# Liozou/CrystalEnergyGrids.jl

Measured on AMD Instinct MI355X. Metric: grid-points/sec, higher is better.
Workload: dtype f64; 1 GPU; CHA_1.4_3b4eeb96 tiled 2x2x3 (11664 atoms) x 256^3 grid, Ar probe LJ + real-space Ewald; grid_points=16777216, framework_atoms=11664, lattice_images=37460, mode=fused, algo=culled, parallelism=x-slab sharding over 1 GPU(s)

## Files before the change

### crystalenergygrids.jl_amd/csrc/ceg_kernels.hip

```cpp
#include <type_traits>

#include "ceg_internal.h"
#include "ceg_math.h"
#include "ceg_minimage.h"

namespace ceg {

struct Accum {
    double v, d1x, d1y, d1z, d2xy, d2xz, d2yz, d3;
};

__device__ __forceinline__ void accum_zero(Accum& a)
{
    a.v = a.d1x = a.d1y = a.d1z = a.d2xy = a.d2xz = a.d2yz = a.d3 = 0.0;
}

__device__ __forceinline__ void accum_add(Accum& a, double v, double p1, double p2, double p3,
                                          double dx, double dy, double dz)
{
    a.v += v;
    a.d1x += p1 * dx;
    a.d1y += p1 * dy;
    a.d1z += p1 * dz;
    const double d13 = dx * dz;
    a.d2xy += p2 * (dx * dy);
    a.d2xz += p2 * d13;
    a.d2yz += p2 * (dy * dz);
    a.d3 += p3 * d13 * dy;
}

__device__ __forceinline__ double grid_coord(int i, double size, int dims, double shift)
{
#pragma clang fp contract(off)
    return __dadd_rn(__ddiv_rn(__dmul_rn((double)i, size), (double)dims), shift);
}

__device__ __attribute__((noinline)) double exp_out_of_line(double x) { return exp(x); }

template <bool LJONLY = false, bool COLD = false>
__device__ __forceinline__ void vdw_terms(const DevRule* __restrict__ rules, int rb, int re, double r2,
                                          double& v_out, double& p1_out, double& p2_out, double& p3_out)
{
    double v = 0.0, p1 = 0.0, p2 = 0.0, p3 = 0.0;
    for (int t = rb; t < re; ++t) {
        const int kind = rules[t].kind;
        const double q0 = rules[t].p0, q1 = rules[t].p1, q2 = rules[t].p2, sh = rules[t].shift;
        double tv, t1 = 0.0, t2 = 0.0, t3 = 0.0;
        if (LJONLY || kind == CEG_LENNARDJONES) {
            const double inv = 1.0 / r2;
            const double s = q1 * inv;
            const double x6 = s * s * s;
            const double inv2 = inv * inv;
            tv = 4.0 * q0 * x6 * (x6 - 1.0);
            t1 = 24.0 * q0 * (x6 * (1.0 - 2.0 * x6)) * inv;
            t2 = 96.0 * q0 * (x6 * (7.0 * x6 - 2.0)) * inv2;
            t3 = 384.0 * q0 * (x6 * (5.0 - 28.0 * x6)) * (inv2 * inv2);
        } else if (kind == CEG_BUCKINGHAM) {
            const double A = q0, B = q1, C = q2;
            const double r4 = r2 * r2;
            const double r = sqrt(r2);
            const double r6 = r4 * r2;
            const double x6 = C / r6;
            const double xe = A * (COLD ? exp_out_of_line(-B * r) : exp(-B * r));
            tv = xe - x6;
            t1 = -B * xe / r + 6.0 * x6 / r2;
            t2 = -48.0 * x6 / r4 + B * xe * (1.0 + B * r) / (r2 * r);
            t3 = -(3.0 * B * r + B * B * r2 + 3.0) * B * xe * r / r6 + 480.0 * C / (r6 * r6);
        } else {
            tv = (r2 < q0) ? __builtin_huge_val() : 0.0;
        }
        v += tv - sh;
        p1 += t1;
        p2 += t2;
        p3 += t3;
    }
    v_out = v; p1_out = p1; p2_out = p2; p3_out = p3;
}

__device__ __forceinline__ void ewald_terms(double alpha, double charge, double r2,
                                            double& v, double& p1, double& p2, double& p3)
{
    const double inv_sqrtpi = 0.56418958354775628695;
    const double r = sqrt(r2);
    const double r3 = r2 * r;
    const double r5 = r3 * r2;
    const double r2a2 = r2 * (alpha * alpha);
    const double er2a2 = 2.0 * alpha * r * exp(-r2a2) * inv_sqrtpi;
    const double erfar = erfc(alpha * r);
    v = charge * erfar / r;
    p1 = -charge * (er2a2 + erfar) / r3;
    p2 = charge * (er2a2 * (3.0 + 2.0 * r2a2) + 3.0 * erfar) / r5;
    p3 = charge * (-er2a2 * (15.0 + 10.0 * r2a2 + 4.0 * (r2a2 * r2a2)) - 15.0 * erfar) / (r5 * r2);
}

__device__ __forceinline__ void ewald_terms_poly(double alpha, double charge, double r2,
                                                 double& v, double& p1, double& p2, double& p3)
{
    const double inv_sqrtpi = 0.56418958354775628695;
    const double r = sqrt(r2);
    const double r3 = r2 * r;
    const double r5 = r3 * r2;
    const double r2a2 = r2 * (alpha * alpha);
    const double E = fast_exp_neg(-r2a2);
    const double er2a2 = 2.0 * alpha * r * E * inv_sqrtpi;
    const double erfar = E * erfcx_poly(alpha * r);
    v = charge * erfar / r;
    p1 = -charge * (er2a2 + erfar) / r3;
    p2 = charge * (er2a2 * (3.0 + 2.0 * r2a2) + 3.0 * erfar) / r5;
    p3 = charge * (-er2a2 * (15.0 + 10.0 * r2a2 + 4.0 * (r2a2 * r2a2)) - 15.0 * erfar) / (r5 * r2);
}

__device__ __attribute__((noinline)) double4 ewald_terms_poly_call(double alpha, double charge, double r2)
{
    double v, p1, p2, p3;
    ewald_terms_poly(alpha, charge, r2, v, p1, p2, p3);
    return make_double4(v, p1, p2, p3);
}
__device__ __attribute__((noinline)) double4 lj_terms_call(const DevRule* __restrict__ rules, int rb, int re, double r2)
{
    double v, p1, p2, p3;
    vdw_terms<true, true>(rules, rb, re, r2, v, p1, p2, p3);
    return make_double4(v, p1, p2, p3);
}

__device__ __forceinline__ double clamp_julia(double x, double lo, double hi)
{
    return (x > hi) ? hi : ((x < lo) ? lo : x);
}

__device__ __forceinline__ void store_gridpoint(float* __restrict__ out, int64_t idx, int64_t cs,
                                                const double* delta, double lambda, double thr, Accum a)
{
#pragma clang fp contract(off)
    if (a.v > thr) {
        a.v = 2.0 * thr;
        a.d1x = clamp_julia(a.d1x, -thr, thr);
        a.d1y = clamp_julia(a.d1y, -thr, thr);
        a.d1z = clamp_julia(a.d1z, -thr, thr);
        a.d2xy = a.d2xz = a.d2yz = 0.0;
        a.d3 = 0.0;
    }
    const double D1 = delta[0], D2 = delta[1], D3 = delta[2];
    out[idx] = (float)__dmul_rn(a.v, lambda);
    out[idx + cs] = (float)__dmul_rn(__dmul_rn(a.d1x, D1), lambda);
    out[idx + 2 * cs] = (float)__dmul_rn(__dmul_rn(a.d1y, D2), lambda);
    out[idx + 3 * cs] = (float)__dmul_rn(__dmul_rn(a.d1z, D3), lambda);
    out[idx + 4 * cs] = (float)__dmul_rn(__dmul_rn(a.d2xy, __dmul_rn(D1, D2)), lambda);
    out[idx + 5 * cs] = (float)__dmul_rn(__dmul_rn(a.d2xz, __dmul_rn(D1, D3)), lambda);
    out[idx + 6 * cs] = (float)__dmul_rn(__dmul_rn(a.d2yz, __dmul_rn(D2, D3)), lambda);
    out[idx + 7 * cs] = (float)__dmul_rn(__dmul_rn(a.d3, __dmul_rn(__dmul_rn(D1, D2), D3)), lambda);
}

__device__ __forceinline__ void gridpoint8(float r[8], const double* delta, double lambda, double thr, Accum a)
{
#pragma clang fp contract(off)
    if (a.v > thr) {
        a.v = 2.0 * thr;
        a.d1x = clamp_julia(a.d1x, -thr, thr);
        a.d1y = clamp_julia(a.d1y, -thr, thr);
        a.d1z = clamp_julia(a.d1z, -thr, thr);
        a.d2xy = a.d2xz = a.d2yz = 0.0;
        a.d3 = 0.0;
    }
    const double D1 = delta[0], D2 = delta[1], D3 = delta[2];
    r[0] = (float)__dmul_rn(a.v, lambda);
    r[1] = (float)__dmul_rn(__dmul_rn(a.d1x, D1), lambda);
    r[2] = (float)__dmul_rn(__dmul_rn(a.d1y, D2), lambda);
    r[3] = (float)__dmul_rn(__dmul_rn(a.d1z, D3), lambda);
    r[4] = (float)__dmul_rn(__dmul_rn(a.d2xy, __dmul_rn(D1, D2)), lambda);
    r[5] = (float)__dmul_rn(__dmul_rn(a.d2xz, __dmul_rn(D1, D3)), lambda);
    r[6] = (float)__dmul_rn(__dmul_rn(a.d2yz, __dmul_rn(D2, D3)), lambda);
    r[7] = (float)__dmul_rn(__dmul_rn(a.d3, __dmul_rn(__dmul_rn(D1, D2), D3)), lambda);
}

typedef float ceg_v4f __attribute__((ext_vector_type(4)));
__device__ __forceinline__ void store_float4_unaligned(float* dst, float4 v)
{
    const ceg_v4f u = {v.x, v.y, v.z, v.w};
    asm volatile("global_store_dwordx4 %0, %1, off" : : "v"(dst), "v"(u) : "memory");
}

__device__ __forceinline__ void store_raw(double* __restrict__ out, int64_t p, const Accum& a)
{
    double* o = out + 8 * p;
    o[0] = a.v;  o[1] = a.d1x;  o[2] = a.d1y;  o[3] = a.d1z;
    o[4] = a.d2xy;  o[5] = a.d2xz;  o[6] = a.d2yz;  o[7] = a.d3;
}

// ... 128 lines not shown
           : (mode == 2 && vdwk >= 2 && ewk) ? CEG_WAVES_FUSED_BUCK
           : (mode == 2 && vdwk == 1 && ewk) ? CEG_WAVES_FUSED_LJ
           : (mode == 0 && vdwk == 1)      ? CEG_WAVES_VDW_LJ
           : (mode == 0 && vdwk >= 2)      ? CEG_WAVES_VDW_BUCK
           : (mode == 1 && ewk)            ? CEG_WAVES_COULOMB
                                           : CEG_WAVES;
}
#ifndef CEG_NW_EW2
#define CEG_NW_EW2 8
#endif
constexpr int culled_nw(int mode, int vdwk, int ewk, int np = 1)
{
    return np > 1 ? (mode == 2 ? CEG_NW_MULTI_FUSED : CEG_WG / 64)
                  : ((mode != 0 && ewk == 2) || (mode != 1 && vdwk == 3)) ? CEG_NW_EW2 : CEG_WG / 64;
}
[[maybe_unused]] constexpr double R_EXACT2 = CEG_R_EXACT2;
static_assert(ERFCX_TAB_N == CEG_ERFCX_TAB_N, "table size mismatch");
constexpr int META_SIMPLE = 1 << 24;
constexpr int META_HASVDW = 1 << 25;
constexpr int META_BUCK = 1 << 26;
constexpr int META_KINDMASK = (1 << 24) - 1;

struct __attribute__((aligned(16))) Quad { double x, y, z, w; };
struct __attribute__((aligned(16))) CandRec {
    Quad xyzq;
    Quad lj;
    int32_t meta;
    int32_t atom;
    int32_t _pad[2];
};

template <int MODE, bool FASTEW, bool LJSLOW, bool EWSCALED, bool BKSCALED, int NP, int UNI = 0, bool DOV = true, bool DOC = true, typename Rec>
__device__ __forceinline__ void slow_pairs(const PlanConst* __restrict__ pc, unsigned long long cands, int lane,
                                           double px, double py, double pz,
                                           const Rec* s_rec,
                                           const unsigned long long* s_odd,
                                           Accum* avm, const int32_t* probe_idx, Accum& ac, double& smallest_d2)
{
    Accum& av = avm[0];
    const Geom& g = pc->g;
    while (cands != 0ull) {
        const int q = __builtin_ctzll(cands);
        cands &= cands - 1ull;
        const unsigned long long lanes = s_odd[q];
        if (!((lanes >> lane) & 1ull)) continue;
        const int mt = s_rec[q].meta;
        const double4 O = pc->ib.atoms[s_rec[q].atom];
        double dx = px - O.x, dy = py - O.y, dz = pz - O.z;
        const double r2 = periodic_distance2_literal(g, dx, dy, dz);
        if (r2 >= g.cutoff2) continue;
        if constexpr (NP > 1) {
            if (DOV && (mt & META_HASVDW)) {
                const int kd = mt & META_KINDMASK;
#pragma unroll
                for (int p = 0; p < NP; ++p) {
                    const RuleTable& rtp = pc->rtm[probe_idx[p]];
                    const int rb = rtp.offset[kd], re = rtp.offset[kd + 1];
                    if (re == rb) continue;
                    const double4 T = lj_terms_call(rtp.rules, rb, re, r2);
                    accum_add(avm[p], T.x, T.y * (-1.0 / 6.0), T.z * (1.0 / 48.0), T.w * (-1.0 / 480.0), dx, dy, dz);
                }
            }
        } else if (MODE != MODE_COULOMB && (mt & META_HASVDW)) {
            const int kd = mt & META_KINDMASK;
            double v, p1, p2, p3;
            vdw_terms<LJSLOW, true>(pc->rt.rules, pc->rt.offset[kd], pc->rt.offset[kd + 1], r2, v, p1, p2, p3);
            if (UNI) {
                v *= pc->uni_sv; p1 *= pc->uni_s1; p2 *= pc->uni_s2; p3 *= pc->uni_s3;
            } else if (LJSLOW) {
                p1 *= -1.0 / 6.0; p2 *= 1.0 / 48.0; p3 *= -1.0 / 480.0;
            }
            if (BKSCALED) {
                v *= pc->bk_invC; p1 *= pc->bk_s1; p2 *= pc->bk_s2; p3 *= pc->bk_s3;
            }
            accum_add(av, v, p1, p2, p3, dx, dy, dz);
        }
        if (MODE != MODE_VDW && DOC) {
            smallest_d2 = fmin(smallest_d2, r2);
            double v, p1, p2, p3;
            if constexpr (NP > 1) {
                const double4 T = ewald_terms_poly_call(g.alpha, O.w, r2);
                v = T.x; p1 = T.y; p2 = T.z; p3 = T.w;
            } else if (FASTEW)
                ewald_terms_poly(g.alpha, O.w, r2, v, p1, p2, p3);
            else
                ewald_terms(g.alpha, O.w, r2, v, p1, p2, p3);
            if (UNI == 2) {
                v *= pc->uni_inv_q; p1 *= pc->uni_inv_q; p2 *= pc->uni_qs2; p3 *= pc->uni_qs3;
            } else if (EWSCALED) {
                p2 *= 1.0 / 3.0; p3 *= 1.0 / 15.0;
            }
            accum_add(ac, v, p1, p2, p3, dx, dy, dz);
        }
    }
}

__device__ __forceinline__ int mad_u24(int a, int b, int c)
{
    int r;
    asm("v_mad_u32_u24 %0, %1, %2, %3" : "=v"(r) : "v"(a), "v"(b), "s"(c));
    return r;
}

__device__ __forceinline__ double uniform(double x)
{
    int lo = __double2loint(x), hi = __double2hiint(x);
    asm("" : "+v"(lo));
    asm("" : "+v"(hi));
    return __hiloint2double(__builtin_amdgcn_readfirstlane(hi), __builtin_amdgcn_readfirstlane(lo));
}

__device__ __forceinline__ double wave_min(double x)
{
#pragma unroll
    for (int o = 32; o > 0; o >>= 1) x = fmin(x, __shfl_xor(x, o));
    return x;
}
__device__ __forceinline__ double wave_max(double x)
{
#pragma unroll
    for (int o = 32; o > 0; o >>= 1) x = fmax(x, __shfl_xor(x, o));
    return x;
}

static_assert(sizeof(CandRec) == 80, "candidate record layout");
struct __attribute__((aligned(16))) CandRecS {
    Quad xyzq;
    int32_t meta;
    int32_t atom;
    int32_t _pad[2];
};
static_assert(sizeof(CandRecS) == 48, "candidate record layout");
template <int NP>
struct __attribute__((aligned(16))) CandRecM {
    Quad xyzq;
    double ljm[3 * NP + (NP & 1)];
    int32_t meta;
    int32_t atom;
    int32_t _pad[2];
};
static_assert(sizeof(CandRecM<2>) == 96 && sizeof(CandRecM<3>) == 128 && sizeof(CandRecM<4>) == 144, "candidate record layout");
template <int NP> __device__ __forceinline__ Quad lj_record(const CandRecM<NP>& r, int p) { return Quad{r.ljm[3 * p], 0.0, r.ljm[3 * p + 1], r.ljm[3 * p + 2]}; }
__device__ __forceinline__ Quad lj_record(const CandRec& r, int) { return r.lj; }
__device__ __forceinline__ Quad lj_record(const CandRecS&, int) { return Quad{0.0, 0.0, 0.0, 0.0}; }
template <int NP> __device__ __forceinline__ void set_lj_record(CandRecM<NP>& r, int p, Quad q) { r.ljm[3 * p] = q.x; r.ljm[3 * p + 1] = q.z; r.ljm[3 * p + 2] = q.w; }
__device__ __forceinline__ void set_lj_record(CandRec& r, int, Quad q) { r.lj = q; }
__device__ __forceinline__ void set_lj_record(CandRecS&, int, Quad) {}

template <int MODE, bool POINTS, int VDWK, int EWK, int NP = 1>
__global__ __launch_bounds__(64 * culled_nw(MODE, VDWK, EWK, NP), culled_waves(MODE, VDWK, EWK, NP)) void k_culled(const PlanConst* __restrict__ pc, Output out, Points pts,
                                                              int tiles_j, int tiles_k, int64_t ntiles)
{
    static_assert(NP >= 1 && NP <= CEG_MAX_PROBES && (NP == 1 || (VDWK == 1 && !POINTS && EWK == 2 && MODE != MODE_COULOMB)), "multi-probe variant");
    constexpr bool MULTI = NP > 1;
    constexpr bool FASTEW = EWK != 0;
    constexpr bool EW2 = EWK == 2 && MODE != MODE_VDW;
    constexpr int WG = 64 * culled_nw(MODE, VDWK, EWK, NP);
    constexpr bool BK2 = VDWK == 3 && MODE != MODE_COULOMB;
    constexpr bool UNI = vdwk_uniform(VDWK) && MODE != MODE_COULOMB;
    constexpr bool UNIQ = VDWK == 5 && MODE == MODE_FUSED && EWK == 2;
    static_assert(!vdwk_uniform(VDWK) || (NP == 1 && MODE != MODE_COULOMB && (VDWK == 4 || UNIQ)), "uniform variants");
    constexpr int NW = WG / 64;
    constexpr bool HAS_LJ = !MULTI && (VDWK == 1 || VDWK == 2) && MODE != MODE_COULOMB;
    using Rec = std::conditional_t<MULTI, CandRecM<NP>, std::conditional_t<HAS_LJ, CandRec, CandRecS>>;
    __shared__ __attribute__((aligned(16))) Rec s_rec_all[NW][64];
    __shared__ int32_t s_rowstart_all[NW][64];
    __shared__ int32_t s_rowprefix_all[NW][66];
    __shared__ unsigned long long s_odd_all[NW][64];
    __shared__ __attribute__((aligned(16))) double s_erfcx[EW2 ? 2 : ERFCX_TAB_N * 6];
    constexpr int EW2_LS = (NP == 1) ? CEG_EW2_LDS_STRIDE : CEG_EW2_STRIDE;
    __shared__ __attribute__((aligned(16))) double s_ew2[EW2 ? CEG_EW2_NI_MAX * EW2_LS : 2];
    __shared__ __attribute__((aligned(16))) double s_bk2[BK2 ? CEG_BK2_NI_MAX * CEG_BK2_STRIDE : 2];
    __shared__ double s_exp2[64];
    __shared__ int32_t s_org[NW][4];

    const int wave = __builtin_amdgcn_readfirstlane(threadIdx.x >> 6);
    Rec* s_rec = s_rec_all[wave];
    int32_t* s_rowstart = s_rowstart_all[wave];
    int32_t* s_rowprefix = s_rowprefix_all[wave];
    unsigned long long* s_odd = s_odd_all[wave];

    constexpr bool FASTVDW = VDWK != 0;
    if (EW2) {
        const int nt = pc->ew2_ni * CEG_EW2_STRIDE;
        for (int t = threadIdx.x; t < nt; t += WG) s_ew2[(t / CEG_EW2_STRIDE) * EW2_LS + t % CEG_EW2_STRIDE] = pc->ew2_tab[t];
    } else if (FASTEW && MODE != MODE_VDW) {
        for (int t = threadIdx.x; t < ERFCX_TAB_N * 6; t += WG) s_erfcx[t] = pc->erfcx_tab[t];
    }
    if (BK2) {
        const int nt = pc->bk2_ni * CEG_BK2_STRIDE;
        for (int t = threadIdx.x; t < nt; t += WG) s_bk2[t] = pc->bk2_tab[t];
    }
    if ((FASTEW && !EW2 && MODE != MODE_VDW) || (VDWK == 2 && MODE != MODE_COULOMB))
        if (threadIdx.x < 64) s_exp2[threadIdx.x] = pc->exp2_tab[threadIdx.x];
    __syncthreads();
    const int64_t tile_raw = (int64_t)blockIdx.x * NW + wave;
    const bool active = tile_raw < ntiles;
    const int64_t tile = active ? tile_raw : ntiles - 1;

    const Geom& g = pc->g;
    const ImageBins& ib = pc->ib;
    const RuleTable& rt = pc->rt;
    const int lane = threadIdx.x & 63;
    const double cutoff2 = g.cutoff2;
    const double r_exact2 = pc->r_exact2;
    const double alpha = g.alpha;
    const int32_t ortho = g.ortho;
    const double safemin2 = g.safemin2;

    int i = 0, j = 0, k = 0;
    int i0 = 0, j0 = 0, k0 = 0;
    int64_t pidx = 0;
    bool valid;
    double px, py, pz;
    if (POINTS) {
        pidx = tile * 64 + lane;
        valid = active && pidx < pts.n;
        const int64_t tt = valid ? pidx : (pts.n - 1);
        px = pts.xyz[3 * tt]; py = pts.xyz[3 * tt + 1]; pz = pts.xyz[3 * tt + 2];
    } else {
        const int tj = (int)((tile / tiles_k) % tiles_j);
        const int ti = (int)(tile / ((int64_t)tiles_k * tiles_j));
        const int nq = (tiles_k + NW - 1) / NW;
        const int tk = (int)((tile % tiles_k + (int64_t)NW * ((ti + (out.i_begin >> 2) + tj) % nq)) % tiles_k);
        i0 = out.i_begin + 4 * ti; j0 = 4 * tj; k0 = 4 * tk;
        if (lane == 0) {
            s_org[wave][0] = active ? i0 : -1;
            s_org[wave][1] = j0;
            s_org[wave][2] = k0;
        }
        i = i0 + (lane >> 4);
        j = j0 + ((lane >> 2) & 3);
        k = k0 + (lane & 3);
        valid = active && (i < out.i_end) && (j <= g.dims[1]) && (k <= g.dims[2]);
        const int ci = i < out.i_end ? i : out.i_end - 1;
        const int cj = j <= g.dims[1] ? j : g.dims[1];
        const int ck = k <= g.dims[2] ? k : g.dims[2];
        px = grid_coord(ci, g.size[0], g.dims[0], g.shift[0]);
        py = grid_coord(cj, g.size[1], g.dims[1], g.shift[1]);
        pz = grid_coord(ck, g.size[2], g.dims[2], g.shift[2]);
    }

    const double blx = uniform(wave_min(px)), bhx = uniform(wave_max(px));
    const double bly = uniform(wave_min(py)), bhy = uniform(wave_max(py));
    const double blz = uniform(wave_min(pz)), bhz = uniform(wave_max(pz));
    const double cx = uniform(0.5 * (blx + bhx)), cy = uniform(0.5 * (bly + bhy)), cz = uniform(0.5 * (blz + bhz));
    const double hx = uniform(0.5 * (bhx - blx)), hy = uniform(0.5 * (bhy - bly)), hz = uniform(0.5 * (bhz - blz));
    const double rc2 = uniform(cutoff2 * (1.0 + 1e-9) + 1e-9);
    const double rc = uniform(sqrt(rc2));

    auto bin_of = [&](double x, int ax) -> int {
        int b = (int)floor((x - ib.lo[ax]) * ib.inv_bin[ax]);
        b = b < 0 ? 0 : b;
        return b >= ib.nb[ax] ? ib.nb[ax] - 1 : b;
    };
    const int bx0 = bin_of(blx - rc, 0), bx1 = bin_of(bhx + rc, 0);
    const int by0 = bin_of(bly - rc, 1), by1 = bin_of(bhy + rc, 1);
    const int nry = by1 - by0 + 1;
    const int nrows = active ? (bx1 - bx0 + 1) * nry : 0;
    const float inv_nry = __int_as_float(__builtin_amdgcn_readfirstlane(__float_as_int(1.0f / (float)nry)));

    Accum avm[NP], ac;
#pragma unroll
    for (int p = 0; p < NP; ++p) accum_zero(avm[p]);
    Accum& av = avm[0];
    accum_zero(ac);
    double smallest_d2 = __builtin_huge_val();
    const double band_cut = 1e-9 * cutoff2;
    const double alpha2 = pc->alpha2;
    const bool stale_possible = !ortho && safemin2 < cutoff2;
    const double cut_hi = uniform(cutoff2 + band_cut);
    const double reg_hi = uniform(stale_possible ? fmin(cutoff2 - band_cut, safemin2 * (1.0 - 1e-9)) : cutoff2 - band_cut);
    const double erf_inv_h = pc->erfcx_inv_h, erf_mx0 = pc->erfcx_mx0_inv_h;
    const int hi_lo = __builtin_amdgcn_readfirstlane(__double2hiint(r_exact2) + (__double2loint(r_exact2) != 0 ? 1 : 0));
    const int hi_top = __builtin_amdgcn_readfirstlane(__double2hiint(reg_hi));
    const unsigned hi_span = hi_top > hi_lo ? (unsigned)(hi_top - hi_lo) : 0u;
    const int hi_cut = __builtin_amdgcn_readfirstlane(__double2hiint(cut_hi));
    const double int_lo = uniform(r_exact2 * (1.0 + 4e-6)), int_hi = uniform(reg_hi * (1.0 - 4e-6));
    const int ew2_off = EW2 ? __builtin_amdgcn_readfirstlane(-pc->ew2_base * (EW2_LS * 8)) : 0;
    int ew2_stride = EW2_LS * 8;
    asm volatile("" : "+v"(ew2_stride));
    const double ew_k3 = pc->ew_k3, ew_k15 = pc->ew_k15;
    const bool all_simple = __builtin_amdgcn_readfirstlane(pc->all_simple) != 0;
    const int bk2_off = BK2 ? __builtin_amdgcn_readfirstlane(-pc->bk2_base * (CEG_BK2_STRIDE * 8)) : 0;
    int bk2_stride = CEG_BK2_STRIDE * 8;
    asm volatile("" : "+v"(bk2_stride));
    const double uni_s6 = UNI ? uniform(pc->uni_s6) : 0.0, uni_k1 = UNI ? uniform(pc->uni_k1) : 0.0;
    const double uni_k2 = UNI ? uniform(pc->uni_k2) : 0.0, uni_k3 = UNI ? uniform(pc->uni_k3) : 0.0;
    const double uni_inv_q = UNIQ ? uniform(pc->uni_inv_q) : 0.0;
    int uni_count = 0;
    int uni_count_all = 0;
    const double bk_B = pc->bk_B, bk_nshift = pc->bk_nshift, bk_c1 = pc->bk_c1, bk_c2 = pc->bk_c2, bk_c3 = pc->bk_c3, bk_c4 = pc->bk_c4;

    for (int rbase = 0; rbase < nrows; rbase += 64) {
        int count = 0, start = 0;
        const int r = rbase + lane;
        if (r < nrows) {
            const int rq = (int)(((float)r + 0.5f) * inv_nry);
            const int bx = bx0 + rq, by = by0 + (r - rq * nry);
            const double colx0 = ib.lo[0] + bx * ib.bin[0], colx1 = colx0 + ib.bin[0];
            const double coly0 = ib.lo[1] + by * ib.bin[1], coly1 = coly0 + ib.bin[1];
            const double gx = fmax(0.0, fmax(blx - colx1, colx0 - bhx));
            const double gy = fmax(0.0, fmax(bly - coly1, coly0 - bhy));
            const double dxy2 = gx * gx + gy * gy;
            if (dxy2 < rc2) {
                const double zr = sqrt(rc2 - dxy2);
                const int bz0 = bin_of(blz - zr, 2), bz1 = bin_of(bhz + zr, 2);
                const int64_t rowbase = ((int64_t)bx * ib.nb[1] + by) * ib.nb[2];
                start = ib.bin_start[rowbase + bz0];
                count = ib.bin_start[rowbase + bz1 + 1] - start;
            }
        }
        int ln = lane;
        asm volatile("" : "+v"(ln));
        int incl = count;
#pragma unroll
        for (int o = 1; o < 64; o <<= 1) {
            const int up = __builtin_amdgcn_ds_bpermute((ln - o) << 2, incl);
            if (ln >= o) incl += up;
        }
        __builtin_amdgcn_wave_barrier();
        s_rowstart[ln] = start;
        s_rowprefix[ln + 1] = incl;
        if (ln == 0) s_rowprefix[0] = 0;
        __builtin_amdgcn_wave_barrier();
        const int total = __builtin_amdgcn_readfirstlane(s_rowprefix[64]);

        for (int cbase = 0; cbase < total; cbase += 64) {
            const int t = cbase + lane;
            bool keep = false, interior = false;
            double4 P = make_double4(0, 0, 0, 0);
            double4 LJ = make_double4(0, 0, 0, 0);
            double4 LJM[NP];
#pragma unroll
            for (int p = 0; p < NP; ++p) LJM[p] = make_double4(0, 0, 0, 0);
            int meta = 0, aidx = 0;
            if (t < total) {
                int lo = 0, hi = 64;
#pragma unroll
                for (int s = 0; s < 6; ++s) {
                    const int mid = (lo + hi) >> 1;
                    if (s_rowprefix[mid] <= t) lo = mid; else hi = mid;
                }
                const int img = s_rowstart[lo] + (t - s_rowprefix[lo]);
                P = ib.xyzq[img];
                aidx = ib.atom[img];
                const int kw = ib.kind ? ib.kind[img] : -1;
                const int kd = kw < 0 ? -1 : (kw & META_KINDMASK);
                const double qx = fmax(0.0, fabs(cx - P.x) - hx);
                const double qy = fmax(0.0, fabs(cy - P.y) - hy);
                const double qz = fmax(0.0, fabs(cz - P.z) - hz);
                const double dmin2 = qx * qx + qy * qy + qz * qz;
                keep = dmin2 < rc2;
                const double fx = fabs(cx - P.x) + hx, fy = fabs(cy - P.y) + hy, fz = fabs(cz - P.z) + hz;
                interior = dmin2 > int_lo && (fx * fx + fy * fy + fz * fz) < int_hi;
                bool hasvdw = false;
                int vclass = 0;
                if (MODE != MODE_COULOMB && kd >= 0) {
                    hasvdw = (kw & META_HASVDW) != 0;
                    if constexpr (MULTI) {
                        if (hasvdw && keep) {
#pragma unroll
                            for (int p = 0; p < NP; ++p) {
                                const FastVdw F = pc->fastm[out.probe_idx[p]][kd];
                                LJM[p] = make_double4(F.p0, F.p1, F.p2, F.shift);
                            }
                        }
                    } else if (FASTVDW && VDWK != 3 && !UNI && hasvdw && keep) {
                        const FastVdw F = pc->fastvdw[kd];
                        LJ = make_double4(F.p0, F.p1, F.p2, F.shift);
                        vclass = F.cls;
                    }
                }
                if (MODE == MODE_VDW) keep = keep && hasvdw;
                bool simple = g.diag != 0 || (!POINTS && all_simple);
                if (!simple && keep) {
                    const double* I = g.invmat;
                    const double ux = cx - P.x, uy = cy - P.y, uz = cz - P.z;
                    const double f0 = I[0] * ux + I[3] * uy + I[6] * uz;
                    const double f1 = I[1] * ux + I[4] * uy + I[7] * uz;
                    const double f2 = I[2] * ux + I[5] * uy + I[8] * uz;
                    const double e0 = fabs(I[0]) * hx + fabs(I[3]) * hy + fabs(I[6]) * hz + 1e-9;
                    const double e1 = fabs(I[1]) * hx + fabs(I[4]) * hy + fabs(I[7]) * hz + 1e-9;
                    const double e2 = fabs(I[2]) * hx + fabs(I[5]) * hy + fabs(I[8]) * hz + 1e-9;
                    simple = (fabs(f0) + e0 < 0.5) && (fabs(f1) + e1 < 0.5) && (fabs(f2) + e2 < 0.5);
                }
                meta = (kd & META_KINDMASK) | (simple ? META_SIMPLE : 0) | (hasvdw ? META_HASVDW : 0) |
                       (vclass == 2 ? META_BUCK : 0);
            }
#ifdef CEG_SKIP_TESTS
            keep = keep && (P.x == 12345.678);
#endif
            const bool simple_c = (meta & META_SIMPLE) != 0;
            const bool withv = MODE != MODE_COULOMB && (meta & META_HASVDW) != 0;
            const bool ks = keep && simple_c;
            const unsigned long long mask_vi = __builtin_amdgcn_ballot_w64(ks && withv && interior);
            const unsigned long long mask_vb = __builtin_amdgcn_ballot_w64(ks && withv && !interior);
            const unsigned long long mask_ni = __builtin_amdgcn_ballot_w64(ks && !withv && interior);
            const unsigned long long mask_nb = __builtin_amdgcn_ballot_w64(ks && !withv && !interior);
            const unsigned long long mask_x = __builtin_amdgcn_ballot_w64(keep && !simple_c);
            const int nvi = __popcll(mask_vi), nv = nvi + __popcll(mask_vb), nni = nv + __popcll(mask_ni), nreg = nni + __popcll(mask_nb),
                      nkeep = nreg + __popcll(mask_x);
            __builtin_amdgcn_wave_barrier();
            if (keep) {
                const unsigned long long mine = !simple_c ? mask_x : (withv ? (interior ? mask_vi : mask_vb) : (interior ? mask_ni : mask_nb));
                const int first = !simple_c ? nreg : (withv ? (interior ? 0 : nvi) : (interior ? nv : nni));
                const int slot = first + __builtin_amdgcn_mbcnt_hi((unsigned)(mine >> 32), __builtin_amdgcn_mbcnt_lo((unsigned)mine, 0));
                s_rec[slot].xyzq = Quad{P.x, P.y, P.z, (UNIQ && !withv) ? mul_sc(P.w, uni_inv_q) : P.w};
                if constexpr (MULTI) {
#pragma unroll
                    for (int p = 0; p < NP; ++p) set_lj_record(s_rec[slot], p, Quad{LJM[p].x, LJM[p].y, LJM[p].z, LJM[p].w});
                } else if constexpr (HAS_LJ) s_rec[slot].lj = Quad{LJ.x, LJ.y, LJ.z, LJ.w};
                s_rec[slot].meta = meta;
                s_rec[slot].atom = aidx;
            }
            __builtin_amdgcn_wave_barrier();

            unsigned long long slow = 0ull;
            auto pair_body = [&](const int q, auto with_vdw_tag, auto interior_tag) __attribute__((always_inline)) {
                constexpr bool WITH_VDW = decltype(with_vdw_tag)::value;
                constexpr bool INTERIOR = decltype(interior_tag)::value;
                const Quad A = s_rec[q].xyzq;
                double dx = px - A.x, dy = py - A.y, dz = pz - A.z;
                const double r2 = dx * dx + dy * dy + dz * dz;
                const int hi = __double2hiint(r2);
                if constexpr (!INTERIOR) {
                    const unsigned long long m_in = __builtin_amdgcn_uicmp((unsigned)(hi - hi_lo), hi_span, 36);
                    const unsigned long long oddlanes = __builtin_amdgcn_sicmp(hi, hi_cut, 41) & ~m_in;
                    if (oddlanes != 0ull) {
                        slow |= 1ull << q;
                        if (lane == 0) s_odd[q] = oddlanes;
                    }
                    if (!((unsigned)(hi - hi_lo) < hi_span)) return;
                }

                const double dxy = dx * dy, dxz = dx * dz, dyz = dy * dz;
                const double dxyz = dxz * dy;
                double rr = 0.0, rinv = 0.0, inv = 0.0;
                constexpr bool NEED_SQRT = ((VDWK == 2 || VDWK == 3) && MODE != MODE_COULOMB) || (EWK == 1 && MODE != MODE_VDW);
                if (NEED_SQRT) {
                    fast_sqrt_rsqrt(r2, rr, rinv);
                    inv = rinv * rinv;
                } else if (FASTVDW || EW2) {
                    inv = fast_rcp(r2);
                }
                int key = 0;
                double t = 0.0;
                static_assert(CEG_BK2_SHIFT == CEG_EW2_SHIFT, "the Buckingham table shares the interval key of the Ewald tables");
                if (EW2 || (BK2 && WITH_VDW)) {
                    key = (int)((unsigned)hi >> CEG_EW2_SHIFT);
                    t = r2 - __hiloint2double(hi & (int)(0xffffffffu << CEG_EW2_SHIFT), 0);
                }
                if constexpr (WITH_VDW && MULTI) {
                    const double inv2 = inv * inv;
                    const double y3 = inv2 * inv;
                    const double inv4 = inv2 * inv2;
#pragma unroll
                    for (int p = 0; p < NP; ++p) {
                        const Quad L = lj_record(s_rec[q], p);
                        const double x6 = L.z * y3;
                        const double w = L.x * x6;
                        const double u = w * x6;
                        const double v = (u - w) - L.w;
                        const double p1 = __builtin_fma(u, 2.0, -w) * inv;
                        const double p2 = fms_vsv(u, 3.5, w) * inv2;
                        const double p3 = fms_vsv(u, 5.6, w) * inv4;
                        Accum& a = avm[p];
                        a.v += v;
                        a.d1x = __builtin_fma(p1, dx, a.d1x);
                        a.d1y = __builtin_fma(p1, dy, a.d1y);
                        a.d1z = __builtin_fma(p1, dz, a.d1z);
                        a.d2xy = __builtin_fma(p2, dxy, a.d2xy);
                        a.d2xz = __builtin_fma(p2, dxz, a.d2xz);
                        a.d2yz = __builtin_fma(p2, dyz, a.d2yz);
                        a.d3 = __builtin_fma(p3, dxyz, a.d3);
                    }
                } else if constexpr (WITH_VDW) {
                    double v, p1, p2, p3;
                    if constexpr (UNI) {
                        const double inv2 = inv * inv;
                        const double z = inv2 * inv;
                        const double a = z * z;
                        v = fms_vsv(a, uni_s6, z);
// ... 393 lines not shown
```

### crystalenergygrids.jl_amd/csrc/ceg_math.h

```cpp
#pragma once

#include <hip/hip_runtime.h>

namespace ceg {

__device__ __forceinline__ double fma_sc(double p, double t, double c)
{
    double r;
    asm("v_fma_f64 %0, %1, %2, %3" : "=v"(r) : "v"(p), "v"(t), "s"(c));
    return r;
}

__device__ __forceinline__ double add_sc(double a, double c)
{
    double r;
    asm("v_add_f64 %0, %1, %2" : "=v"(r) : "v"(a), "s"(c));
    return r;
}
__device__ __forceinline__ double fma2_sc(double a, double c)
{
    double r;
    asm("v_fma_f64 %0, %1, 2.0, %2" : "=v"(r) : "v"(a), "s"(c));
    return r;
}
__device__ __forceinline__ double fma4_sc(double a, double c)
{
    double r;
    asm("v_fma_f64 %0, %1, 4.0, %2" : "=v"(r) : "v"(a), "s"(c));
    return r;
}

__device__ __forceinline__ double mul_sc(double a, double c)
{
    double r;
    asm("v_mul_f64 %0, %1, %2" : "=v"(r) : "v"(a), "s"(c));
    return r;
}

__device__ __forceinline__ double fma_vsv(double a, double b, double c)
{
    double r;
    asm("v_fma_f64 %0, %1, %2, %3" : "=v"(r) : "v"(a), "s"(b), "v"(c));
    return r;
}

__device__ __forceinline__ double fms_vsv(double a, double b, double c)
{
    double r;
    asm("v_fma_f64 %0, %1, %2, -%3" : "=v"(r) : "v"(a), "s"(b), "v"(c));
    return r;
}

__device__ __forceinline__ double min_nonan(double a, double b)
{
    double r;
    asm("v_min_f64 %0, %1, %2" : "=v"(r) : "v"(a), "v"(b));
    return r;
}

__device__ __forceinline__ void fast_sqrt_rsqrt(double a, double& s, double& rs)
{
    const double y = __builtin_amdgcn_rsq(a);
    const double t = a * y;
    const double e = __builtin_fma(-t, y, 1.0);
    double p;
    asm("v_fma_f64 %0, %1, %2, 0.5" : "=v"(p) : "v"(e), "s"(0.375));
    const double q = y * e;
    rs = __builtin_fma(q, p, y);
    s = a * rs;
}

#ifndef CEG_RCP_ITERS
#define CEG_RCP_ITERS 1
#endif
__device__ __forceinline__ double fast_rcp(double a)
{
    double y = __builtin_amdgcn_rcp(a);
#pragma unroll
    for (int it = 0; it < CEG_RCP_ITERS; ++it) {
        const double e = __builtin_fma(-a, y, 1.0);
        y = __builtin_fma(y, e, y);
    }
    return y;
}

__device__ __forceinline__ double fast_exp_neg(double y)
{
    const double log2e = 1.4426950408889634074;
    const double ln2_hi = 6.93147180369123816490e-01;
    const double ln2_lo = 1.90821492927058770002e-10;
    const double k = __builtin_rint(y * log2e);
    double r = __builtin_fma(-k, ln2_hi, y);
    r = __builtin_fma(-k, ln2_lo, r);
    double p = 1.6059043836821613e-10;
    p = fma_sc(p, r, 2.08767569878681e-09);
    p = fma_sc(p, r, 2.505210838544172e-08);
    p = fma_sc(p, r, 2.755731922398589e-07);
    p = fma_sc(p, r, 2.7557319223985893e-06);
    p = fma_sc(p, r, 2.48015873015873e-05);
    p = fma_sc(p, r, 1.984126984126984e-04);
    p = fma_sc(p, r, 1.388888888888889e-03);
    p = fma_sc(p, r, 8.333333333333333e-03);
    p = fma_sc(p, r, 4.1666666666666664e-02);
    p = fma_sc(p, r, 1.6666666666666666e-01);
    p = __builtin_fma(p, r, 0.5);
    p = __builtin_fma(p, r, 1.0);
    p = __builtin_fma(p, r, 1.0);
    return __builtin_ldexp(p, (int)k);
}

constexpr int ERFCX_TAB_N = 128;

__device__ __forceinline__ double erfcx_tab(const double* __restrict__ tab, double x, double inv_h, double mx0_inv_h)
{
    const double u = __builtin_fma(x, inv_h, mx0_inv_h);
    unsigned idx = (unsigned)u;
    idx = idx < (unsigned)(ERFCX_TAB_N - 1) ? idx : (unsigned)(ERFCX_TAB_N - 1);
    const double sl = __builtin_amdgcn_fract(u);
    const double2* c = reinterpret_cast<const double2*>(tab + idx * 6);
    const double2 c01 = c[0], c23 = c[1], c45 = c[2];
    double p = __builtin_fma(c45.y, sl, c45.x);
    p = __builtin_fma(p, sl, c23.y);
    p = __builtin_fma(p, sl, c23.x);
    p = __builtin_fma(p, sl, c01.y);
    p = __builtin_fma(p, sl, c01.x);
    return p;
}

__device__ __forceinline__ double exp_neg_tab(const double* __restrict__ exp2_tab, double y)
{
    const double c64_log2e = 92.33248261689366;
    const double ln2_64_hi = 0.01083042469326756;
    const double ln2_64_lo = 2.9815858269852933e-12;
    const double kf = __builtin_rint(y * c64_log2e);
    const int k = (int)kf;
    double r = __builtin_fma(-kf, ln2_64_hi, y);
    r = __builtin_fma(-kf, ln2_64_lo, r);
    const double T = exp2_tab[k & 63];
    double q = fma_vsv(r, 8.3333333333333332e-03, 4.1666666666666664e-02);
    q = fma_sc(q, r, 1.6666666666666666e-01);
    q = __builtin_fma(q, r, 0.5);
    q = __builtin_fma(q, r, 1.0);
    const double pr = q * r;
    return __builtin_ldexp(__builtin_fma(T, pr, T), k >> 6);
}

constexpr double ERFCX_XMAX = 5.0;

__device__ __forceinline__ double erfcx_poly(double x)
{
    const double u = 2.0 * fast_rcp(2.0 + x);
    const double t = __builtin_fma(u, 2.8, -1.8);
    double p = -8.831938387231295e-11;
    p = fma_sc(p, t, -4.135667802654713e-11);
    p = fma_sc(p, t, 1.3922900473941904e-09);
    p = fma_sc(p, t, -2.706262020862157e-09);
    p = fma_sc(p, t, -5.482959765234865e-09);
    p = fma_sc(p, t, 4.311416522498039e-08);
    p = fma_sc(p, t, -8.16041092885496e-08);
    p = fma_sc(p, t, -2.2284362873574516e-07);
    p = fma_sc(p, t, 1.6349752166110725e-06);
    p = fma_sc(p, t, -1.9074493734062743e-06);
    p = fma_sc(p, t, -1.641101524432363e-05);
    p = fma_sc(p, t, 6.508546403940596e-05);
    p = fma_sc(p, t, 0.0001235891242710475);
    p = fma_sc(p, t, -0.0012713100507524312);
    p = fma_sc(p, t, -0.0016962844625334375);
    p = fma_sc(p, t, 0.028193785197004564);
    p = fma_sc(p, t, 0.15791059062700571);
    p = fma_sc(p, t, 0.41766221044962965);
    p = fma_sc(p, t, 0.3990292854009171);
    return p;
}

__device__ __forceinline__ void sincos_2pi(double u, double& s, double& c)
{
    u -= rint(u);
    const double k = rint(4.0 * u);
    const double v = __builtin_fma(k, -0.25, u);
    const double x = v * 6.283185307179586476925;
    const double z = x * x;
    double ps = 1.58962301576546568060e-10;
    ps = __builtin_fma(ps, z, -2.50507477628578072866e-8);
    ps = __builtin_fma(ps, z, 2.75573136213857245213e-6);
    ps = __builtin_fma(ps, z, -1.98412698295895385996e-4);
    ps = __builtin_fma(ps, z, 8.33333333332211858878e-3);
    ps = __builtin_fma(ps, z, -1.66666666666666307295e-1);
    const double sinx = __builtin_fma(x * z, ps, x);
    double pc = -1.13585365213876817300e-11;
    pc = __builtin_fma(pc, z, 2.08757008419747316778e-9);
    pc = __builtin_fma(pc, z, -2.75573141792967388112e-7);
    pc = __builtin_fma(pc, z, 2.48015872888517045348e-5);
    pc = __builtin_fma(pc, z, -1.38888888888730564116e-3);
    pc = __builtin_fma(pc, z, 4.16666666666665929218e-2);
    const double cosx = __builtin_fma(z * z, pc, __builtin_fma(z, -0.5, 1.0));
    const int q = (int)k & 3;
    const double a = (q & 1) ? cosx : sinx, b = (q & 1) ? sinx : cosx;
    s = (q & 2) ? -a : a;
    c = ((q + 1) & 2) ? -b : b;
}

}
```

Baseline: 1.308 billion grid-points/s.

## Replace per-candidate binary row search with incremental wave-wide row stepping

Row lookup for candidate images switches from a six-step binary search over shared-memory prefix sums to an incremental walk that reads prefix values from lanes, with row starts pre-offset so the image index is a plain add. Ballot masks are built from four base ballots instead of five compound ones, and the non-points bounding box takes only lanes 0 and 63 instead of a full wave reduction. The Ewald polynomial constants in the hot path are now loaded through scalar-register inline asm, which aims to cut literal and register pressure. The row-stepping loop is serial per chunk and depends on uniform readlane, and the volatile asm constants may block scheduling.

```diff
diff --git a/crystalenergygrids.jl_amd/csrc/ceg_kernels.hip b/crystalenergygrids.jl_amd/csrc/ceg_kernels.hip
--- a/crystalenergygrids.jl_amd/csrc/ceg_kernels.hip
+++ b/crystalenergygrids.jl_amd/csrc/ceg_kernels.hip
@@ -2,6 +2,7 @@
 
 #include "ceg_internal.h"
 #include "ceg_math.h"
+#include "ceg_rowlookup.h"
 #include "ceg_minimage.h"
 
 namespace ceg {
@@ -93,17 +94,18 @@
     p3 = charge * (-er2a2 * (15.0 + 10.0 * r2a2 + 4.0 * (r2a2 * r2a2)) - 15.0 * erfar) / (r5 * r2);
 }
 
+template <bool COLD = false>
 __device__ __forceinline__ void ewald_terms_poly(double alpha, double charge, double r2,
                                                  double& v, double& p1, double& p2, double& p3)
 {
-    const double inv_sqrtpi = 0.56418958354775628695;
+    constexpr double inv_sqrtpi = 0.56418958354775628695;
     const double r = sqrt(r2);
     const double r3 = r2 * r;
     const double r5 = r3 * r2;
     const double r2a2 = r2 * (alpha * alpha);
-    const double E = fast_exp_neg(-r2a2);
-    const double er2a2 = 2.0 * alpha * r * E * inv_sqrtpi;
-    const double erfar = E * erfcx_poly(alpha * r);
+    const double E = fast_exp_neg<COLD>(-r2a2);
+    const double er2a2 = 2.0 * alpha * r * E * CEG_KC(COLD, inv_sqrtpi);
+    const double erfar = E * erfcx_poly<COLD>(alpha * r);
     v = charge * erfar / r;
     p1 = -charge * (er2a2 + erfar) / r3;
     p2 = charge * (er2a2 * (3.0 + 2.0 * r2a2) + 3.0 * erfar) / r5;
@@ -398,13 +400,13 @@
                 const double4 T = ewald_terms_poly_call(g.alpha, O.w, r2);
                 v = T.x; p1 = T.y; p2 = T.z; p3 = T.w;
             } else if (FASTEW)
-                ewald_terms_poly(g.alpha, O.w, r2, v, p1, p2, p3);
+                ewald_terms_poly<true>(g.alpha, O.w, r2, v, p1, p2, p3);
             else
                 ewald_terms(g.alpha, O.w, r2, v, p1, p2, p3);
             if (UNI == 2) {
                 v *= pc->uni_inv_q; p1 *= pc->uni_inv_q; p2 *= pc->uni_qs2; p3 *= pc->uni_qs3;
             } else if (EWSCALED) {
-                p2 *= 1.0 / 3.0; p3 *= 1.0 / 15.0;
+                p2 *= CEG_KC(true, 1.0 / 3.0); p3 *= CEG_KC(true, 1.0 / 15.0);
             }
             accum_add(ac, v, p1, p2, p3, dx, dy, dz);
         }
@@ -424,6 +426,11 @@
     asm("" : "+v"(lo));
     asm("" : "+v"(hi));
     return __hiloint2double(__builtin_amdgcn_readfirstlane(hi), __builtin_amdgcn_readfirstlane(lo));
+}
+
+__device__ __forceinline__ double lane_value(double x, int L)
+{
+    return __hiloint2double(__builtin_amdgcn_readlane(__double2hiint(x), L), __builtin_amdgcn_readlane(__double2loint(x), L));
 }
 
 __device__ __forceinline__ double wave_min(double x)
@@ -557,9 +564,22 @@
         pz = grid_coord(ck, g.size[2], g.dims[2], g.shift[2]);
     }
 
-    const double blx = uniform(wave_min(px)), bhx = uniform(wave_max(px));
-    const double bly = uniform(wave_min(py)), bhy = uniform(wave_max(py));
-    const double blz = uniform(wave_min(pz)), bhz = uniform(wave_max(pz));
+    double blx_, bhx_, bly_, bhy_, blz_, bhz_;
+    if (POINTS) {
+        blx_ = wave_min(px); bhx_ = wave_max(px);
+        bly_ = wave_min(py); bhy_ = wave_max(py);
+        blz_ = wave_min(pz); bhz_ = wave_max(pz);
+    } else {
+        const double ax = lane_value(px, 0), bx = lane_value(px, 63);
+        const double ay = lane_value(py, 0), by = lane_value(py, 63);
+        const double az = lane_value(pz, 0), bz = lane_value(pz, 63);
+        blx_ = fmin(ax, bx); bhx_ = fmax(ax, bx);
+        bly_ = fmin(ay, by); bhy_ = fmax(ay, by);
+        blz_ = fmin(az, bz); bhz_ = fmax(az, bz);
+    }
+    const double blx = uniform(blx_), bhx = uniform(bhx_);
+    const double bly = uniform(bly_), bhy = uniform(bhy_);
+    const double blz = uniform(blz_), bhz = uniform(bhz_);
     const double cx = uniform(0.5 * (blx + bhx)), cy = uniform(0.5 * (bly + bhy)), cz = uniform(0.5 * (blz + bhz));
     const double hx = uniform(0.5 * (bhx - blx)), hy = uniform(0.5 * (bhy - bly)), hz = uniform(0.5 * (bhz - blz));
     const double rc2 = uniform(cutoff2 * (1.0 + 1e-9) + 1e-9);
@@ -636,11 +656,11 @@
             if (ln >= o) incl += up;
         }
         __builtin_amdgcn_wave_barrier();
-        s_rowstart[ln] = start;
+        s_rowstart[ln] = start - (incl - count);
         s_rowprefix[ln + 1] = incl;
-        if (ln == 0) s_rowprefix[0] = 0;
         __builtin_amdgcn_wave_barrier();
-        const int total = __builtin_amdgcn_readfirstlane(s_rowprefix[64]);
+        const int total = __builtin_amdgcn_readlane(incl, 63);
+        int row = 0;
 
         for (int cbase = 0; cbase < total; cbase += 64) {
             const int t = cbase + lane;
@@ -651,14 +671,16 @@
 #pragma unroll
             for (int p = 0; p < NP; ++p) LJM[p] = make_double4(0, 0, 0, 0);
             int meta = 0, aidx = 0;
+            bool simple = false, hasvdw = false;
+            int lo;
+            {
+                const int kk = row + 1 + lane;
+                const int pv = s_rowprefix[kk < 64 ? kk : 64];
+                const int row0 = row;
+                row = row_lookup_step(row0, cbase, t, [&](int k) { return __builtin_amdgcn_readlane(pv, k - row0 - 1); }, lo);
+            }
             if (t < total) {
-                int lo = 0, hi = 64;
-#pragma unroll
-                for (int s = 0; s < 6; ++s) {
-                    const int mid = (lo + hi) >> 1;
-                    if (s_rowprefix[mid] <= t) lo = mid; else hi = mid;
-                }
-                const int img = s_rowstart[lo] + (t - s_rowprefix[lo]);
+                const int img = s_rowstart[lo] + t;
                 P = ib.xyzq[img];
                 aidx = ib.atom[img];
                 const int kw = ib.kind ? ib.kind[img] : -1;
@@ -670,7 +692,6 @@
                 keep = dmin2 < rc2;
                 const double fx = fabs(cx - P.x) + hx, fy = fabs(cy - P.y) + hy, fz = fabs(cz - P.z) + hz;
                 interior = dmin2 > int_lo && (fx * fx + fy * fy + fz * fz) < int_hi;
-                bool hasvdw = false;
                 int vclass = 0;
                 if (MODE != MODE_COULOMB && kd >= 0) {
                     hasvdw = (kw & META_HASVDW) != 0;
@@ -689,7 +710,7 @@
                     }
                 }
                 if (MODE == MODE_VDW) keep = keep && hasvdw;
-                bool simple = g.diag != 0 || (!POINTS && all_simple);
+                simple = g.diag != 0 || (!POINTS && all_simple);
                 if (!simple && keep) {
                     const double* I = g.invmat;
                     const double ux = cx - P.x, uy = cy - P.y, uz = cz - P.z;
@@ -707,14 +728,17 @@
 #ifdef CEG_SKIP_TESTS
             keep = keep && (P.x == 12345.678);
 #endif
-            const bool simple_c = (meta & META_SIMPLE) != 0;
-            const bool withv = MODE != MODE_COULOMB && (meta & META_HASVDW) != 0;
-            const bool ks = keep && simple_c;
-            const unsigned long long mask_vi = __builtin_amdgcn_ballot_w64(ks && withv && interior);
-            const unsigned long long mask_vb = __builtin_amdgcn_ballot_w64(ks && withv && !interior);
-            const unsigned long long mask_ni = __builtin_amdgcn_ballot_w64(ks && !withv && interior);
-            const unsigned long long mask_nb = __builtin_amdgcn_ballot_w64(ks && !withv && !interior);
-            const unsigned long long mask_x = __builtin_amdgcn_ballot_w64(keep && !simple_c);
+            const bool simple_c = simple;
+            const bool withv = MODE != MODE_COULOMB && hasvdw;
+            const unsigned long long m_keep = __builtin_amdgcn_ballot_w64(keep);
+            const unsigned long long m_ks = __builtin_amdgcn_ballot_w64(keep && simple);
+            const unsigned long long m_v = __builtin_amdgcn_ballot_w64(withv);
+            const unsigned long long m_i = __builtin_amdgcn_ballot_w64(interior);
+            const unsigned long long mask_vi = m_ks & m_v & m_i;
+            const unsigned long long mask_vb = m_ks & m_v & ~m_i;
+            const unsigned long long mask_ni = m_ks & ~m_v & m_i;
+            const unsigned long long mask_nb = m_ks & ~m_v & ~m_i;
+            const unsigned long long mask_x = m_keep & ~m_ks;
             const int nvi = __popcll(mask_vi), nv = nvi + __popcll(mask_vb), nni = nv + __popcll(mask_ni), nreg = nni + __popcll(mask_nb),
                       nkeep = nreg + __popcll(mask_x);
             __builtin_amdgcn_wave_barrier();
diff --git a/crystalenergygrids.jl_amd/csrc/ceg_math.h b/crystalenergygrids.jl_amd/csrc/ceg_math.h
--- a/crystalenergygrids.jl_amd/csrc/ceg_math.h
+++ b/crystalenergygrids.jl_amd/csrc/ceg_math.h
@@ -10,6 +10,17 @@
     asm("v_fma_f64 %0, %1, %2, %3" : "=v"(r) : "v"(p), "v"(t), "s"(c));
     return r;
 }
+
+template <unsigned LO, unsigned HI>
+__device__ __forceinline__ double literal_f64_here()
+{
+    int lo, hi;
+    asm volatile("s_mov_b32 %0, %1" : "=s"(lo) : "n"((int)LO));
+    asm volatile("s_mov_b32 %0, %1" : "=s"(hi) : "n"((int)HI));
+    return __hiloint2double(hi, lo);
+}
+#define CEG_F64_BITS(C) __builtin_bit_cast(unsigned long long, (double)(C))
+#define CEG_KC(COLD, C) ((COLD) ? ::ceg::literal_f64_here<(unsigned)(CEG_F64_BITS(C) & 0xffffffffull), (unsigned)(CEG_F64_BITS(C) >> 32)>() : (double)(C))
 
 __device__ __forceinline__ double add_sc(double a, double c)
 {
@@ -84,25 +95,26 @@
     return y;
 }
 
+template <bool COLD = false>
 __device__ __forceinline__ double fast_exp_neg(double y)
 {
-    const double log2e = 1.4426950408889634074;
-    const double ln2_hi = 6.93147180369123816490e-01;
-    const double ln2_lo = 1.90821492927058770002e-10;
-    const double k = __builtin_rint(y * log2e);
-    double r = __builtin_fma(-k, ln2_hi, y);
-    r = __builtin_fma(-k, ln2_lo, r);
-    double p = 1.6059043836821613e-10;
-    p = fma_sc(p, r, 2.08767569878681e-09);
-    p = fma_sc(p, r, 2.505210838544172e-08);
-    p = fma_sc(p, r, 2.755731922398589e-07);
-    p = fma_sc(p, r, 2.7557319223985893e-06);
-    p = fma_sc(p, r, 2.48015873015873e-05);
-    p = fma_sc(p, r, 1.984126984126984e-04);
-    p = fma_sc(p, r, 1.388888888888889e-03);
-    p = fma_sc(p, r, 8.333333333333333e-03);
-    p = fma_sc(p, r, 4.1666666666666664e-02);
-    p = fma_sc(p, r, 1.6666666666666666e-01);
+    constexpr double log2e = 1.4426950408889634074;
+    constexpr double ln2_hi = 6.93147180369123816490e-01;
+    constexpr double ln2_lo = 1.90821492927058770002e-10;
+    const double k = __builtin_rint(y * CEG_KC(COLD, log2e));
+    double r = __builtin_fma(-k, CEG_KC(COLD, ln2_hi), y);
+    r = __builtin_fma(-k, CEG_KC(COLD, ln2_lo), r);
+    double p = CEG_KC(COLD, 1.6059043836821613e-10);
+    p = fma_sc(p, r, CEG_KC(COLD, 2.08767569878681e-09));
+    p = fma_sc(p, r, CEG_KC(COLD, 2.505210838544172e-08));
+    p = fma_sc(p, r, CEG_KC(COLD, 2.755731922398589e-07));
+    p = fma_sc(p, r, CEG_KC(COLD, 2.7557319223985893e-06));
+    p = fma_sc(p, r, CEG_KC(COLD, 2.48015873015873e-05));
+    p = fma_sc(p, r, CEG_KC(COLD, 1.984126984126984e-04));
+    p = fma_sc(p, r, CEG_KC(COLD, 1.388888888888889e-03));
+    p = fma_sc(p, r, CEG_KC(COLD, 8.333333333333333e-03));
+    p = fma_sc(p, r, CEG_KC(COLD, 4.1666666666666664e-02));
+    p = fma_sc(p, r, CEG_KC(COLD, 1.6666666666666666e-01));
     p = __builtin_fma(p, r, 0.5);
     p = __builtin_fma(p, r, 1.0);
     p = __builtin_fma(p, r, 1.0);
@@ -147,29 +159,30 @@
 
 constexpr double ERFCX_XMAX = 5.0;
 
+template <bool COLD = false>
 __device__ __forceinline__ double erfcx_poly(double x)
 {
     const double u = 2.0 * fast_rcp(2.0 + x);
-    const double t = __builtin_fma(u, 2.8, -1.8);
-    double p = -8.831938387231295e-11;
-    p = fma_sc(p, t, -4.135667802654713e-11);
-    p = fma_sc(p, t, 1.3922900473941904e-09);
-    p = fma_sc(p, t, -2.706262020862157e-09);
-    p = fma_sc(p, t, -5.482959765234865e-09);
-    p = fma_sc(p, t, 4.311416522498039e-08);
-    p = fma_sc(p, t, -8.16041092885496e-08);
-    p = fma_sc(p, t, -2.2284362873574516e-07);
-    p = fma_sc(p, t, 1.6349752166110725e-06);
-    p = fma_sc(p, t, -1.9074493734062743e-06);
-    p = fma_sc(p, t, -1.641101524432363e-05);
-    p = fma_sc(p, t, 6.508546403940596e-05);
-    p = fma_sc(p, t, 0.0001235891242710475);
-    p = fma_sc(p, t, -0.0012713100507524312);
-    p = fma_sc(p, t, -0.0016962844625334375);
-    p = fma_sc(p, t, 0.028193785197004564);
-    p = fma_sc(p, t, 0.15791059062700571);
-    p = fma_sc(p, t, 0.41766221044962965);
-    p = fma_sc(p, t, 0.3990292854009171);
+    const double t = __builtin_fma(u, CEG_KC(COLD, 2.8), CEG_KC(COLD, -1.8));
+    double p = CEG_KC(COLD, -8.831938387231295e-11);
+    p = fma_sc(p, t, CEG_KC(COLD, -4.135667802654713e-11));
+    p = fma_sc(p, t, CEG_KC(COLD, 1.3922900473941904e-09));
+    p = fma_sc(p, t, CEG_KC(COLD, -2.706262020862157e-09));
+    p = fma_sc(p, t, CEG_KC(COLD, -5.482959765234865e-09));
+    p = fma_sc(p, t, CEG_KC(COLD, 4.311416522498039e-08));
+    p = fma_sc(p, t, CEG_KC(COLD, -8.16041092885496e-08));
+    p = fma_sc(p, t, CEG_KC(COLD, -2.2284362873574516e-07));
+    p = fma_sc(p, t, CEG_KC(COLD, 1.6349752166110725e-06));
+    p = fma_sc(p, t, CEG_KC(COLD, -1.9074493734062743e-06));
+    p = fma_sc(p, t, CEG_KC(COLD, -1.641101524432363e-05));
+    p = fma_sc(p, t, CEG_KC(COLD, 6.508546403940596e-05));
+    p = fma_sc(p, t, CEG_KC(COLD, 0.0001235891242710475));
+    p = fma_sc(p, t, CEG_KC(COLD, -0.0012713100507524312));
+    p = fma_sc(p, t, CEG_KC(COLD, -0.0016962844625334375));
+    p = fma_sc(p, t, CEG_KC(COLD, 0.028193785197004564));
+    p = fma_sc(p, t, CEG_KC(COLD, 0.15791059062700571));
+    p = fma_sc(p, t, CEG_KC(COLD, 0.41766221044962965));
+    p = fma_sc(p, t, CEG_KC(COLD, 0.3990292854009171));
     return p;
 }
 
diff --git a/crystalenergygrids.jl_amd/csrc/ceg_rowlookup.h b/crystalenergygrids.jl_amd/csrc/ceg_rowlookup.h
--- /dev/null
+++ b/crystalenergygrids.jl_amd/csrc/ceg_rowlookup.h
@@ -0,0 +1,37 @@
+#pragma once
+
+#if defined(__HIPCC__) || defined(__CUDACC__)
+#define CEG_ROWLOOKUP_FN __host__ __device__ __forceinline__
+#else
+#define CEG_ROWLOOKUP_FN inline
+#endif
+
+namespace ceg {
+
+template <class PrefixAt>
+CEG_ROWLOOKUP_FN int row_lookup_search(int t, PrefixAt&& prefix_at)
+{
+    int lo = 0, hi = 64;
+    for (int s = 0; s < 6; ++s) {
+        const int mid = (lo + hi) >> 1;
+        if (prefix_at(mid) <= t) lo = mid; else hi = mid;
+    }
+    return lo;
+}
+
+template <class PrefixAt>
+CEG_ROWLOOKUP_FN int row_lookup_step(int row, int cbase, int t, PrefixAt&& prefix_at, int& lo)
+{
+    const int next_base = cbase + 64;
+    int k = row + 1;
+    lo = row;
+    while (k < 64) {
+        const int s = prefix_at(k);
+        if (s > next_base) break;
+        lo += (s <= t) ? 1 : 0;
+        ++k;
+    }
+    return k - 1;
+}
+
+}
```

New measurement: 1.321 billion grid-points/s, median of 6. About the same (+0.9%).
